# h-walk/PySlice

Hardware: AMD Instinct MI355X
Metric: slice-steps/sec (probes x frames x slices / s), potential + slice loop + exit FFT (higher is better)
Workload: dtype complex64 (f32); 1 GPU; 64-probe STEM grid, 1024x1024 grid, 200 slices, 54 MD frames per GPU (BASELINE configs[2] per-frame work), 106583 atoms, 30 mrad, 100 keV; grid=1024, slices=200, probes=64, parallelism=frames x1, world_size_checked=1, frame_slots=59, frame_batch=4

## Files before the change

### pyslice_amd/csrc/mslice.hip

```cpp
#include <hip/hip_runtime.h>

#include <algorithm>
#include <cmath>
#include <cstdarg>
#include <cstdio>
#include <cstdlib>
#include <cstring>
#include <string>
#include <type_traits>
#include <vector>

#include "../../include/mslice.h"
#include "fft_generic.h"
#include "fft_pow2.h"
#include "rowtm_pass.h"
#include "potential.h"
#include "thermal.h"
#include "phonons.h"
#include "reduce.h"
#include "stream.h"
#include "tacaw_time.h"
#include "tacaw_launch.h"
#include "tacaw_welch.h"
#include "layer_tap.h"
// ... 36 lines not shown
    }
    int reserve(msl_handle* h, size_t count) { return count <= n ? MSL_OK : alloc(h, count); }
};

struct FftPlan {
    int M = 0;
    DevBuf<float2> chirp, bfilt;
    int N = 0;
    int n_stages = 0;
    int radix[MSL_MAX_STAGES] = {0};
    DevBuf<float2> tw;
    bool ok = false;
};

enum LaunchKind { K_ROW = 0, K_COL = 1, K_OTHER = 2, K_NKINDS = 3 };

enum AxisKind { AX_NONE, AX_FOURSTEP, AX_TWO, AX_WAVE2K, AX_MIXED, AX_CONV, AX_CONV2K, AX_CONV4K, AX_GENERIC };

enum PotIfft { PI_LINES, PI_TWO, PI_CHIRPZ, PI_WAVE2K };

struct CzTables { int R = 0; DevBuf<float2> tw, tw2, bf, bw; };

struct EventSet {
    std::vector<hipEvent_t> ev;
    std::vector<int> kind;
    int used = 0;
    bool pending = false;
};

}

struct msl_handle {
    msl_config cfg{};
    hipStream_t stream = nullptr;
    std::string err;
    FftPlan plan_x, plan_y, plan_t;
    int Rx = 0, Ry = 0;
    DevBuf<float2> tw4_x, tw4_y;
    int n_cus = 256;
    int wx = 0, wy = 0, wx0 = 0, wy0 = 0;
    size_t wpix = 0;
    size_t wpitch = 0;
    size_t intensity_ld = 0;
    int bx = 1, by = 1;
    DevBuf<float2> bin_stage;
    DevBuf<float2> st_acc, st_tw; DevBuf<double2> st_s1; DevBuf<double> st_s2; DevBuf<int> st_bins;
    DevBuf<float2> st_ref; bool st_have_ref = false;
    int st_T = 0, st_F = 0; bool st_open = false;
    int64_t intensity_F = 0;
    DevBuf<char> scratch;
    bool onepass = false;
    bool scheme_b = false;
    PotIfft pot_ifft = PI_LINES;
    struct OpDir { AxisKind kind = AX_NONE, base = AX_NONE; int n = 0; int R = 0; DevBuf<float2> mtw, tw, tw2, qf, bw, ptab;
                   CzTables cz; } opx, opy;
    CzTables opt;
    int opt_T = 0;
    DevBuf<float2> tsplit_tw;
    int tsplit_T = 0;
    DevBuf<float> welch_g;
    std::vector<float> welch_g_host;
    DevBuf<float2> psiT, psi0T;
    bool need_psi0T = false;
    int keys_cap = 0;
    struct HostStage { char* buf = nullptr; size_t bytes = 0; hipEvent_t ev = nullptr; bool used = false; } stage[2];
    unsigned stage_pos = 0;
    DevBuf<float2> transT;
    int pitchT = 0;
    int debug_flags_mask = -1;
    int row_pchunk = 0;
    int pitch = 0;
    int FB = 1, cur_batch = 0;
    DevBuf<float2> psi0, psi, trans;
    DevBuf<float> V;
    DevBuf<float> intensity;
    DevBuf<float2> pxt, pyt;
    std::vector<int> layer_block;
    std::vector<int> layer_slices;
    DevBuf<float2> layers;
    float2* wf = nullptr;
    DevBuf<float2> tap, tap_cx, tap_cy;
    bool lr_on = false;
    unsigned lr_what = 0;
    int lr_bx = 1, lr_by = 1, lr_slot = 0, lr_count = 0;
    LrLayout lr_lay;
    DevBuf<float2> lr_block;
    DevBuf<double> lr_stage;
    DevBuf<uint16_t> det_mask;
    DevBuf<float> det_kx, det_ky;
    int det_n = 0, det_wy = 0;
    size_t det_K = 0;
    uint32_t det_amp = 0, det_cx = 0, det_cy = 0;
    DevBuf<uint32_t> pol_order;
    DevBuf<long long> pol_seg;
    int pol_bins = 0;
    size_t pol_K = 0;
    DevBuf<double> diff_out;
    DevBuf<double2> coh_acc;
    int64_t coh_B = 0, coh_K = 0;
    DevBuf<double> img_acc;
    int64_t img_n = 0;
    std::vector<int32_t> sm_h;
    DevBuf<int2> sm_beams;
    DevBuf<float2> sm_S, sm_c;
    int sm_fx = 0, sm_fy = 0, sm_Bm = 0;
    bool sm_open = false, sm_built = false;
// ... 806 lines not shown
            j.in = h->psiT; j.out = h->psi;
            j.trans = h->transT + toff + (size_t)k * npix; j.pl = h->pxt;
            j.in_image_stride = isB; j.out_image_stride = isA; j.in_pitch = h->pitchT; j.out_pitch = h->pitch; j.n_lines = c.ny;
            rc = launch_rowT_dir(h, h->opx, j, K_COL);
        }
        if (rc) return rc;
        if (k < nz - 1) {
            int rp = 0;
            const int order = tap_order((k & 1) ? h->opx : h->opy, j.flags, j.perm_shift, &rp);
            if ((rc = tap_step(h, k, fused_slot, groups, (k & 1) ? h->psi : h->psiT, !(k & 1), order, rp, (k & 1) ? 1 : 0))) return rc;
        }
    }
    if (nz & 1) {
        dim3 grid((c.nx + 31) / 32, (c.ny + 31) / 32, P);
        hipLaunchKernelGGL(transpose_kernel, grid, dim3(256), 0, h->stream, h->psiT, h->psi, c.ny, c.nx, h->pitchT, h->pitch, isB, isA);
        HIPCHK(h, hipGetLastError());
        if ((rc = mark_launch(h, K_OTHER))) return rc;
    }
    if (fused) {
        if (h->Ry) {
            RowJob r = row_job(h, h->psi, P, h->pitch);
            r.do_fft = true;
            if ((rc = launch_row_fast(h, r, K_OTHER))) return rc;
        } else {
            LineArgs r = row_args(h, h->psi, h->psi, P, h->pitch);
            r.fft1 = +1;
            if ((rc = launch_lines(h, h->plan_y, r, K_OTHER))) return rc;
        }
        if ((rc = epilogue_x_pass(h, fused_slot, groups))) return rc;
    }
    count_slice_loop(h, P, groups, fused, 16);
    return MSL_OK;
}

template <int R>
int launch_row2_r(msl_handle* h, Row2Job job, int kind) {
    constexpr int N = R * R, G = 256 / R;
    const size_t lds = (size_t)N * 16 + (size_t)G * R * (R + 1) * 4;
    const int per_cu = std::max(1, std::min(2, (int)((size_t)h->lds_limit / lds)));
    const int grid = chunked_grid(h, job, job.nx / G, (long long)h->n_cus * per_cu);
    hipLaunchKernelGGL(row_pass2_kernel<R>, dim3(grid), dim3(256), lds, h->stream, job);
    HIPCHK(h, hipGetLastError());
    return mark_launch(h, kind);
}

int slice_loop_onepass(msl_handle* h, int fused_slot, int groups, int first_group) {
    if (h->scheme_b) return slice_loop_onepass_b(h, fused_slot, groups, first_group);
    const msl_config& c = h->cfg;
    const int P = c.n_probes * groups, nz = c.nz;
    const size_t toff = (size_t)first_group * c.nz * c.nx * c.ny;
    const size_t npix = (size_t)c.nx * c.ny;
    const long long isA = (long long)c.nx * h->pitch, isB = (long long)c.ny * h->pitchT;
    const bool fused = fused_slot >= 0;
    int rc;
    if (nz == 1)
        HIPCHK(h, hipMemcpyAsync(h->psi, h->psi0, (size_t)P * isA * sizeof(float2), hipMemcpyDeviceToDevice, h->stream));
    if ((rc = begin_timed(h, nz + 2 + (fused ? tap_launches(h) : 0)))) return rc;
    for (int k = 0; k < nz; ++k) {
        const bool last = (k == nz - 1);
        int flags = (k > 0 ? P2_PRE_A : 0) | (!last ? P2_POST_A : 0) | ((last && fused) ? P2_POST_F : 0);
        if (h->debug_flags_mask >= 0) flags &= h->debug_flags_mask;
        if (last) {
            Row2Job j{};
            j.psi = h->psi; j.trans = h->trans + toff + (size_t)k * npix; j.py = h->pyt; j.tw = h->tw4_y;
            j.image_stride = isA; j.pitch = h->pitch; j.nx = c.nx; j.n_images = P; j.flags = flags;
            set_frame_groups(h, j, groups);
            rc = h->Ry == 32 ? launch_row2_r<32>(h, j, K_ROW) : launch_row2_r<16>(h, j, K_ROW);
            if (rc) return rc;
            break;
        }
        const bool along_y = !slice_is_transposed(h, k);
        RowTJob j{};
        if (!dbg_env("MSL_NO_INTERLEAVE") && h->debug_flags_mask < 0) flags |= (k > 0 ? P2_IN_PAIRED : 0) | (k < nz - 2 ? P2_OUT_PAIRED : 0);
        j.flags = flags; j.n_images = P;
        j.perm_shift = ((along_y ? h->Rx : h->Ry) == 32) ? 2 : 1;
        set_frame_groups(h, j, groups);
        if (along_y) {
            j.in = (k == 0) ? h->psi0 : h->psi; j.out = h->psiT;
            j.trans = h->trans + toff + (size_t)k * npix; j.pl = h->pyt; j.tw = h->tw4_y;
            j.in_image_stride = isA; j.out_image_stride = isB; j.in_pitch = h->pitch; j.out_pitch = h->pitchT; j.n_lines = c.nx;
            rc = h->Ry == 32 ? launch_rowT_r<32>(h, j, K_ROW) : launch_rowT_r<16>(h, j, K_ROW);
        } else {
            j.in = (k == 0) ? h->psi0T : h->psiT; j.out = h->psi;
            j.trans = h->transT + toff + (size_t)k * npix; j.pl = h->pxt; j.tw = h->tw4_x;
            j.in_image_stride = isB; j.out_image_stride = isA; j.in_pitch = h->pitchT; j.out_pitch = h->pitch; j.n_lines = c.ny;
            rc = h->Rx == 32 ? launch_rowT_r<32>(h, j, K_COL) : launch_rowT_r<16>(h, j, K_COL);
        }
        if (rc) return rc;
        const int order = (j.flags & P2_OUT_PAIRED) ? TAP_INTERLEAVED : TAP_NATURAL;
        if ((rc = tap_step(h, k, fused_slot, groups, along_y ? h->psiT : h->psi, along_y, order, 8 << j.perm_shift, along_y ? 0 : 1))) return rc;
    }
    if (fused && (rc = epilogue_x_pass(h, fused_slot, groups))) return rc;
    count_slice_loop(h, P, groups, fused, 16);
    return MSL_OK;
}

int ensure_atoms(msl_handle* h, size_t n, size_t rows) {
    if (rows <= h->atom_cap) return MSL_OK;
    (void)n;
    size_t cap = std::max<size_t>(rows, h->atom_cap * 3 / 2 + 1024);
    int rc;
    if ((rc = h->d_pos.alloc(h, cap * 3)) || (rc = h->d_Z.alloc(h, cap)) || (rc = h->d_key.alloc(h, cap)) || (rc = h->d_order.alloc(h, cap)) ||
        (rc = h->d_u1.alloc(h, cap)) || (rc = h->d_u2.alloc(h, cap))) return rc;
    if ((rc = h->d_ex.alloc(h, cap * (size_t)(h->cfg.nx / 2 + 1))) || (rc = h->d_ey.alloc(h, cap * (size_t)(h->cfg.ny / 2 + 1)))) return rc;
    h->atom_cap = cap;
    return MSL_OK;
}

int slice_loop(msl_handle* h, int fused_slot, int groups, int first_group) {
    if (h->onepass) return slice_loop_onepass(h, fused_slot, groups, first_group);
    const msl_config& c = h->cfg;
    const int P = c.n_probes * groups, nz = c.nz;
    const size_t npix = (size_t)c.nx * c.ny;
    const size_t toff = (size_t)first_group * c.nz * npix;
    HIPCHK(h, hipMemcpyAsync(h->psi, h->psi0, (size_t)P * c.nx * h->pitch * sizeof(float2), hipMemcpyDeviceToDevice, h->stream));
    const bool fused = fused_slot >= 0;
    int rc = begin_timed(h, 2 * nz + 2 + (fused ? tap_launches(h) : 0));
    if (rc) return rc;
    for (int z = 0; z < nz; ++z) {
        const bool last = (z == nz - 1);
        if (h->Ry) {
            RowJob r = row_job(h, h->psi, P, h->pitch);
            r.do_ifft = z > 0; r.trans = h->trans + toff + (size_t)z * npix;
            r.do_fft = (!last || fused); r.py = last ? nullptr : h->pyt;
            set_frame_groups(h, r, groups);
            if ((rc = launch_row_fast(h, r, K_ROW))) return rc;
        } else {
            LineArgs r = row_args(h, h->psi, h->psi, P, h->pitch);
            r.fft1 = (z > 0) ? -1 : 0;
            r.m1_kind = MUL_ARRAY; r.m1 = h->trans + toff + (size_t)z * npix; r.m1_ls = c.ny;
            if (groups > 1) { r.group = c.n_probes; r.m_gs = (long long)c.nz * npix; r.out_gs = (long long)c.n_probes * r.out_is; }
            if (!last) { r.fft2 = +1; r.m2_kind = MUL_VEC; r.m2 = h->pyt; }
            else if (fused) { r.fft2 = +1; }
            if ((rc = launch_lines(h, h->plan_y, r, K_ROW))) return rc;
        }
        if (!last && (rc = tap_step(h, z, fused_slot, groups, h->psi, false, TAP_NATURAL, 8, 2))) return rc;
        if (!last) {
            if (h->Rx) {
                ColJob k = col_job(h, h->psi, h->psi, P, h->pitch, h->pitch);
                k.px = h->pxt; k.flags = COL_FWD | COL_MULPX | COL_INV;
                if ((rc = launch_col_fast(h, k, K_COL))) return rc;
            } else {
                LineArgs k = col_args(h, h->psi, h->psi, P, h->pitch, h->pitch);
                k.fft1 = +1; k.m1_kind = MUL_VEC; k.m1 = h->pxt; k.fft2 = -1;
                if ((rc = launch_lines(h, h->plan_x, k, K_COL))) return rc;
// ... 135 lines not shown
                if (mG == 64) T[n + (n1 % mA) * 2 * mB + 2 * k2 + n1 / mA] = w;
                else T[n + n1 * mB + k2] = w;
            }
        if (mG == 64)
            for (int m = 0; m < mA; ++m) {
                const double a = -2.0 * M_PI * (double)m / (double)(2 * mA);
                T[2 * n + m] = make_float2(1.f, 0.f);
                T[2 * n + mA + m] = make_float2((float)cos(a), (float)sin(a));
            }
        if ((rc = upload(h, o.mtw, T))) return rc;
    }
    switch (o.base) {
    case AX_TWO: {
        std::vector<float2> t(o.R * o.R);
        for (int m = 0; m < o.R * o.R; ++m) {
            const double a = -2.0 * M_PI * (double)m / (double)n;
            t[m] = make_float2((float)cos(a), (float)sin(a));
        }
        if ((rc = make_tw4(h, o.tw, o.R)) || (rc = upload(h, o.tw2, t)) || (rc = o.ptab.alloc(h, (size_t)n))) return rc;
        break;
    }
    case AX_WAVE2K:
        if ((rc = make_wave2k_tables(h, o.tw, o.tw2))) return rc;
        break;
    case AX_CONV:
    case AX_CONV2K:
        if ((rc = make_cz_tables(h, o.cz, n)) || (rc = o.qf.alloc(h, conv_filter_entries(o)))) return rc;
        break;
    case AX_CONV4K: {
        std::vector<float2> wq(2048);
        for (int i = 0; i < 2048; ++i) {
            const double a = -2.0 * M_PI * (double)i / 4096.0;
            wq[i] = make_float2((float)cos(a), (float)sin(a));
        }
        if ((rc = make_wave2k_tables(h, o.tw, o.tw2)) || (rc = upload(h, o.bw, wq)) || (rc = o.qf.alloc(h, conv_filter_entries(o)))) return rc;
        break;
    }
    default:
        break;
    }
    auto conv = [](const msl_handle::OpDir& d) { return d.base == AX_CONV || d.base == AX_CONV2K; };
    if (!conv(o) && conv(other) && n >= 33 && n <= 1024) return make_cz_tables(h, o.cz, n);
    return MSL_OK;
}

PotIfft plan_pot_ifft(const msl_handle* h) {
    if (!h->onepass || h->V) return PI_LINES;
    if (h->opx.base == AX_WAVE2K && h->opy.base == AX_WAVE2K && h->transT) return PI_WAVE2K;
    if (h->transT && h->opx.cz.R && h->opy.cz.R) return PI_CHIRPZ;
    if (h->opx.base == AX_TWO && h->opy.base == AX_TWO) return PI_TWO;
    return PI_LINES;
}

bool pot_half_rows(const msl_handle* h) { return h->pot_ifft != PI_LINES || (h->Rx && h->Ry); }

struct PotGroup {
    int z2s[104], species[104], nsp;
    int64_t n; int32_t ax1, ax2, axs;
    int keys_per_frame;
    int cx, cy; float vscale;
    bool half_rows, sf_stream;
    int g, slot, n_slices, nkeys;
    long long rows, rows_pad;
    float2* TR; float2* TRT;
};

void drop_modes(msl_handle* h) {
    h->have_modes = false;
    h->md_basis.release(); h->md_q.release(); h->md_tau.release(); h->md_W.release(); h->md_C.release();
    h->md_M = h->md_nb = 0;
}

int map_species(msl_handle* h, const int32_t* Z, int64_t n, PotGroup& m) {
    for (int i = 0; i < 104; ++i) m.z2s[i] = -1;
    for (int64_t a = 0; a < n; ++a) {
        if (Z[a] < 1 || Z[a] > 103) return fail(h, MSL_ERR_INVALID, "msl_build_potential: atomic number %d out of 1..103", Z[a]);
        m.z2s[Z[a]] = 0;
    }
    m.nsp = 0;
    for (int z = 1; z <= 103; ++z) if (m.z2s[z] == 0) { m.z2s[z] = m.nsp; m.species[m.nsp++] = z; }
    return MSL_OK;
}

int stage_atoms(msl_handle* h, const PotGroup& p, const double* pos, const int32_t* Z, bool send_maps) {
    msl_handle::HostStage& st = h->stage[h->stage_pos++ & 1];
    if (!st.ev) HIPCHK(h, hipEventCreateWithFlags(&st.ev, hipEventDisableTiming));
    if (st.used) HIPCHK(h, hipEventSynchronize(st.ev));
    const size_t z_bytes = (size_t)p.n * sizeof(int), pos_bytes = (size_t)p.rows * 3 * sizeof(double);
    const size_t off_sp = sizeof p.z2s, off_Z = (off_sp + sizeof p.species + 7) & ~(size_t)7;
    const size_t off_pos = (off_Z + z_bytes + 7) & ~(size_t)7, need = off_pos + pos_bytes;
    if (need > st.bytes) {
        if (st.buf) (void)hipHostFree(st.buf);
        st.buf = nullptr; st.bytes = 0;
        const size_t cap = need + need / 4;
        if (hipHostMalloc((void**)&st.buf, cap, hipHostMallocDefault) != hipSuccess)
            return fail(h, MSL_ERR_NOMEM, "hipHostMalloc(%zu bytes) failed", cap);
        st.bytes = cap;
    }
    memcpy(st.buf + off_pos, pos, pos_bytes);
    if (send_maps) {
        memcpy(st.buf, p.z2s, sizeof p.z2s);
        memcpy(st.buf + off_sp, p.species, sizeof p.species);
        memcpy(st.buf + off_Z, Z, z_bytes);
        HIPCHK(h, hipMemcpyAsync(h->d_z2s, st.buf, sizeof p.z2s, hipMemcpyHostToDevice, h->stream));
        HIPCHK(h, hipMemcpyAsync(h->d_species, st.buf + off_sp, p.nsp * sizeof(int), hipMemcpyHostToDevice, h->stream));
        HIPCHK(h, hipMemcpyAsync(h->d_Z, st.buf + off_Z, z_bytes, hipMemcpyHostToDevice, h->stream));
// ... 529 lines not shown
        static int exchange_ok = -1;
        if (exchange_ok < 0) exchange_ok = rowT_selftest(h->stream);
        if (exchange_ok != 0) return bail(fail(h, MSL_ERR_HIP, "msl_create: the add-tid LDS exchange self-test failed on this device / toolchain (%d values wrong)", exchange_ok));
    }
    if ((rc = make_plan(h, h->plan_x, cfg->nx))) return bail(rc);
    if ((rc = make_plan(h, h->plan_y, cfg->ny))) return bail(rc);
    {
        hipDeviceProp_t prop;
        if (hipGetDeviceProperties(&prop, cfg->device) == hipSuccess && prop.multiProcessorCount > 0) h->n_cus = prop.multiProcessorCount;
    }
    if (cfg->fft_path == 0) {
        int ry = fast_radix(cfg->ny), rx = fast_radix(cfg->nx);
        if (ry && cfg->nx % (256 / ry) == 0) { h->Ry = ry; if ((rc = make_tw4(h, h->tw4_y, ry))) return bail(rc); }
        if (rx && cfg->ny % 16 == 0 && cfg->ny >= 32) { h->Rx = rx; if ((rc = make_tw4(h, h->tw4_x, rx))) return bail(rc); }
        { const char* e = dbg_env("MSL_ROW_PCHUNK"); if (e) h->row_pchunk = atoi(e); }
        allow_lds(h, row_pass_pf_kernel<32>);
        allow_lds(h, row_pass_pf_kernel<16>);
        allow_lds(h, col_pass_kernel<32>);
        allow_lds(h, col_pass_kernel<16>);
    }
    const size_t npix = (size_t)cfg->nx * cfg->ny;
    {
        const char* e = dbg_env("MSL_PITCH_PAD");
        int pad = e ? atoi(e) : 16;
        if (pad < 0 || (pad & 1)) pad = 16;
        h->pitch = cfg->ny + ((h->Rx || h->Ry) ? pad : 0);
    }
    {
        const char* e = dbg_env("MSL_SLICE_PATH");
        const bool want = cfg->fft_path == 0 && !(e && atoi(e) == 2);
        plan_axis_kind(h, h->opx, cfg->nx, cfg->ny, h->Rx, h->plan_x.M, want);
        plan_axis_kind(h, h->opy, cfg->ny, cfg->nx, h->Ry, h->plan_y.M, want);
        if ((rc = make_axis_tables(h, h->opx, h->opy)) || (rc = make_axis_tables(h, h->opy, h->opx))) return bail(rc);
        h->onepass = h->opx.base != AX_NONE && h->opy.base != AX_NONE;
        h->scheme_b = h->onepass && !(h->opx.kind == AX_FOURSTEP && h->opy.kind == AX_FOURSTEP);
        if (h->pitch == cfg->ny && h->onepass) h->pitch = cfg->ny + 16;
        if (h->onepass && (h->pitch & 1)) ++h->pitch;
        if (h->onepass) {
            h->pitchT = cfg->nx + 16 + (cfg->nx & 1);
            if (h->pitch - cfg->ny > 16 && !(cfg->nx & 1)) h->pitchT = cfg->nx + (h->pitch - cfg->ny);
            h->need_psi0T = !h->scheme_b && (cfg->nz % 2 == 0);
        }
        if ((rc = alloc_probe_buffers(h, cfg->n_probes))) return bail(rc);
        if (h->onepass) {
            if ((rc = h->transT.alloc(h, npix * cfg->nz * h->FB))) return bail(rc);
            { const char* ev = dbg_env("MSL_DEBUG_FLAGS_MASK"); if (ev) h->debug_flags_mask = atoi(ev); }
            allow_lds(h, row_pass2_kernel<32>);
            allow_lds(h, row_pass2_kernel<16>);
        }
    }
    if ((rc = h->trans.alloc(h, npix * cfg->nz * h->FB))) return bail(rc);
    if (cfg->keep_potential && (rc = h->V.alloc(h, npix * cfg->nz))) return bail(rc);
    h->pot_ifft = plan_pot_ifft(h);
    if (cfg->n_frames > 0) {
        if ((h->bx > 1 || h->by > 1) && (rc = h->bin_stage.alloc(h, (size_t)h->wx * h->wy * cfg->n_probes * h->FB))) return bail(rc);
        if ((rc = h->layers.alloc(h, layer_block_elems(h)))) return bail(rc);
        h->wf = h->layers;
        if (hipMemsetAsync(h->wf, 0, layer_block_elems(h) * sizeof(float2), h->stream) != hipSuccess)
            return bail(fail(h, MSL_ERR_HIP, "memset failed"));
    }
    if ((rc = h->pxt.alloc(h, (size_t)cfg->nx)) || (rc = h->pyt.alloc(h, (size_t)cfg->ny)) || (rc = h->tap_cx.alloc(h, (size_t)cfg->nx)) ||
        (rc = h->tap_cy.alloc(h, (size_t)cfg->ny)) || (rc = h->d_lo.alloc(h, (size_t)cfg->nz)) || (rc = h->d_hi.alloc(h, (size_t)cfg->nz)) ||
        (rc = h->d_abcd.alloc(h, (size_t)103 * 12)) || (rc = h->d_z2s.alloc(h, (size_t)104)) || (rc = h->d_species.alloc(h, (size_t)104)) ||
        (rc = fill_propagator(h))) return bail(rc);
    *out = h;
    return MSL_OK;
}

int msl_destroy(msl_handle* h) {
    if (!h) return MSL_OK;
    (void)hipSetDevice(h->cfg.device);
    if (h->stream) (void)hipStreamSynchronize(h->stream);
    for (auto& s : h->ring) for (auto e : s.ev) (void)hipEventDestroy(e);
    for (auto& st : h->stage) { if (st.ev) (void)hipEventDestroy(st.ev); if (st.buf) (void)hipHostFree(st.buf); }
    const hipStream_t stream = h->stream;
    delete h;
    if (stream) (void)hipStreamDestroy(stream);
    return MSL_OK;
}

int msl_set_kirkland(msl_handle* h, const double* abcd) {
    if (!h || !abcd) return fail(h, MSL_ERR_INVALID, "msl_set_kirkland: null argument");
    HIPCHK(h, hipSetDevice(h->cfg.device));
    HIPCHK(h, hipMemcpyAsync(h->d_abcd, abcd, 103 * 12 * sizeof(double), hipMemcpyHostToDevice, h->stream));
    HIPCHK(h, hipStreamSynchronize(h->stream));
    h->have_kirkland = true;
    h->n_species = 0;
    h->ff_n = 0;
    return MSL_OK;
}

int msl_set_slices(msl_handle* h, const double* lo, const double* hi) {
    if (!h || !lo || !hi) return fail(h, MSL_ERR_INVALID, "msl_set_slices: null argument");
    for (int s = 0; s < h->cfg.nz; ++s)
        if (!(hi[s] > lo[s]) || (s > 0 && lo[s] < lo[s - 1]))
            return fail(h, MSL_ERR_INVALID, "msl_set_slices: edges must be increasing with hi>lo (slice %d)", s);
    HIPCHK(h, hipSetDevice(h->cfg.device));
    HIPCHK(h, hipMemcpyAsync(h->d_lo, lo, h->cfg.nz * sizeof(double), hipMemcpyHostToDevice, h->stream));
    HIPCHK(h, hipMemcpyAsync(h->d_hi, hi, h->cfg.nz * sizeof(double), hipMemcpyHostToDevice, h->stream));
    HIPCHK(h, hipStreamSynchronize(h->stream));
    h->have_slices = true;
    return MSL_OK;
}

int msl_set_beam(msl_handle* h, double wavelength, double sigma, double dz) {
    if (!h) return fail(h, MSL_ERR_INVALID, "null handle");
// ... 1736 lines not shown
```

### pyslice_amd/csrc/rowt_pass.h

```cpp
#pragma once
#include <type_traits>
#include <utility>
#include <hip/hip_runtime.h>
#include "fft_regs.h"
#include "kernel_util.h"

#ifndef MSL_ABL2
#define MSL_ABL2 0
#endif
#ifndef MSL_TW_LDS
#define MSL_TW_LDS 0
#endif
#ifndef MSL_DIT_LCH
#define MSL_DIT_LCH 8
#endif
#ifndef MSL_DIT_FENCE
#define MSL_DIT_FENCE 0
#endif
#ifndef MSL_STAGGER
#define MSL_STAGGER 4
#endif
#define MSL_IC(x) std::integral_constant<int, (x)>{}

namespace msl {

enum { P2_PRE_A = 1, P2_POST_A = 2, P2_POST_F = 4, P2_IN_PAIRED = 8, P2_OUT_PAIRED = 16 };

struct RowTJob {
    const float2* in;
    float2* out;
    const float2* trans;
    const float2* pl;
    const float2* tw;
    const float2* tw2;
    long long in_image_stride, out_image_stride;
    int in_pitch, out_pitch, n_lines, n_images, flags, pchunk;
    int t_group;
    unsigned t_magic;
    long long t_stride;
    const float2* bf;
    const float2* bw;
    int n_line;
    int perm_shift;
#ifdef MSL_CLOCK
    unsigned long long* clk;
#endif
};

template <typename Job>
__device__ __forceinline__ long long frame_off(const Job& job, int p) {
    if (job.t_group <= 0) return 0;
    const unsigned up = (unsigned)__builtin_amdgcn_readfirstlane(p);
    const unsigned f = job.t_group == 1 ? up : __umulhi(up, job.t_magic);
    return (long long)f * job.t_stride;
}


template <int R>
__device__ __forceinline__ void exchange_addtid(float2 (&v)[R], const float* scratch_base, unsigned wave_scratch, int ln, int lane64) {
    static_assert(64 % R == 0 && R % 4 == 0, "R-lane groups inside one wave; rows are read four floats at a time");
    constexpr int PW = 68;
    if constexpr (MSL_ABL2 & 4) return;
    const float* rd = scratch_base + ln * PW + (lane64 / R) * R;
    asm volatile("s_mov_b32 m0, %0\n\ts_nop 1" :: "s"(wave_scratch) : "memory");
#pragma unroll
    for (int k1 = 0; k1 < R; ++k1) asm volatile("ds_write_addtid_b32 %0 offset:%1" :: "v"(v[k1].x), "n"(k1 * PW * 4) : "memory");
    wave_lds_fence();
#pragma unroll
    for (int g = 0; g < R / 4; ++g) {
        const float4 q = *reinterpret_cast<const float4*>(rd + 4 * g);
        v[4 * g].x = q.x; v[4 * g + 1].x = q.y; v[4 * g + 2].x = q.z; v[4 * g + 3].x = q.w;
    }
    wave_lds_fence();
    asm volatile("s_mov_b32 m0, %0\n\ts_nop 1" :: "s"(wave_scratch) : "memory");
#pragma unroll
    for (int k1 = 0; k1 < R; ++k1) asm volatile("ds_write_addtid_b32 %0 offset:%1" :: "v"(v[k1].y), "n"(k1 * PW * 4) : "memory");
    wave_lds_fence();
#pragma unroll
    for (int g = 0; g < R / 4; ++g) {
        const float4 q = *reinterpret_cast<const float4*>(rd + 4 * g);
        v[4 * g].y = q.x; v[4 * g + 1].y = q.y; v[4 * g + 2].y = q.z; v[4 * g + 3].y = q.w;
    }
    wave_lds_fence();
}

template <int R, bool INV, int WMODE, int STRIDE, int C0, typename TabPtr, int... J>
__device__ __forceinline__ void dit_leaf_chunk(const float2* in, float2* v, TabPtr tab, int ln, std::integer_sequence<int, J...>) {
    constexpr int LR = dit_leaf_radix(R), C = R / LR;
    float2 w[sizeof...(J)][4];
    if constexpr (MSL_ABL2 & 16) {
        ((w[J][0] = tab[ln], w[J][1] = tab[ln], w[J][2] = tab[ln], w[J][3] = tab[ln]), ...);
    } else {
        ((w[J][0] = tab[(C0 + J) * STRIDE + ln], w[J][1] = tab[(C0 + J + C) * STRIDE + ln]), ...);
        if constexpr (LR == 4) ((w[J][2] = tab[(C0 + J + 2 * C) * STRIDE + ln], w[J][3] = tab[(C0 + J + 3 * C) * STRIDE + ln]), ...);
    }
    (dit_leaf<R, INV, WMODE, C0 + J>(in, v, w[J]), ...);
    (pin(v[C0 + J]), ...); (pin(v[C0 + J + C]), ...);
    if constexpr (LR == 4) { (pin(v[C0 + J + 2 * C]), ...); (pin(v[C0 + J + 3 * C]), ...); }
    __builtin_amdgcn_sched_barrier(0);
}
template <int R, bool INV, int WMODE, int STRIDE, int CH, int C0, typename TabPtr>
__device__ __forceinline__ void dit_leaf_chunks(const float2* in, float2* v, TabPtr tab, int ln) {
    if constexpr (C0 < dit_leaf_count(R)) {
        dit_leaf_chunk<R, INV, WMODE, STRIDE, C0>(in, v, tab, ln, std::make_integer_sequence<int, CH>{});
        dit_leaf_chunks<R, INV, WMODE, STRIDE, CH, C0 + CH>(in, v, tab, ln);
    }
}

template <int R, bool INV, int WMODE, int K, int I>
__device__ __forceinline__ void dit_leaves_regs_part(const float2* in, float2* v, const float2* w) {
    if constexpr (I < K) {
        constexpr int LR = dit_leaf_radix(R);
        float2 ww[4];
        ww[0] = w[I]; ww[1] = w[I + K];
        if constexpr (LR == 4) { ww[2] = w[I + 2 * K]; ww[3] = w[I + 3 * K]; }
        dit_leaf<R, INV, WMODE, I>(in, v, ww);
        dit_leaves_regs_part<R, INV, WMODE, K, I + 1>(in, v, w);
    }
}
constexpr int rowT_tw_reg_leaves(int R, int FL) { return (!MSL_TW_LDS && R == 32 && FL >= 0) ? 8 : 0; }
constexpr int ROWT_TW_REG_LCH = 4;

template <int R, int LINES, bool IN_P, bool OUT_P, int FL>
__global__ void __launch_bounds__(LINES * R, (R == 16) ? 3 : 2) rowT_pass_kernel(RowTJob job) {
    constexpr int N = R * R;
    constexpr int NT = LINES * R;
    constexpr int CS = (R * R + 33) / 32 * 32 + 2;
    constexpr int TPS = LINES / 2;
    constexpr int POS_PER_IT = NT / TPS;
    constexpr int NIT = N / POS_PER_IT;
    constexpr int TWK = rowT_tw_reg_leaves(R, FL), LRW = dit_leaf_radix(R);
    constexpr bool TWR = TWK > 0;
    constexpr int LCH0 = TWR ? ROWT_TW_REG_LCH : MSL_DIT_LCH;
    constexpr int LCHL = LCH0 < dit_leaf_count(R) ? LCH0 : dit_leaf_count(R);
    constexpr int FN = MSL_DIT_FENCE;
    static_assert(LINES == 16, "16 lines = 128-byte transposed segments (8 lines / 64 bytes measured 1.6x slower)");
    static_assert(dit_leaf_count(R) % LCHL == 0 && TWK % LCHL == 0 && TWK < dit_leaf_count(R), "whole chunks");
    extern __shared__ __attribute__((aligned(16))) char smem_raw[];
    float2* tw = reinterpret_cast<float2*>(smem_raw);
    float2* pl = tw + N;
    float2* tile = pl + N;
    const int tid = threadIdx.x;
    for (int i = tid; i < N; i += NT) { tw[i] = job.tw[i]; pl[i] = job.pl[i]; }
    __syncthreads();
    const int grp = tid / R, ln = tid % R;
    float2 twr[TWR ? LRW * TWK : 1];
    if constexpr (TWR) {
#pragma unroll
        for (int i = 0; i < LRW * TWK; ++i) twr[i] = tw[((i % TWK) + (i / TWK) * dit_leaf_count(R)) * R + ln];
        pin_all(twr);
    }
    const int q = tid % TPS, r0 = tid / TPS;
    const int l64 = tid & 63;
    float2* myrow = tile + grp * CS;
    const float* wscr = reinterpret_cast<const float*>(tile + (grp - grp % (64 / R)) * CS);
    const unsigned wscr_lds = __builtin_amdgcn_readfirstlane((unsigned)(size_t)(tile + (grp - grp % (64 / R)) * CS));
    const int lblocks = job.n_lines / LINES;
    const int PC = job.pchunk;
    const int pchunks = (job.n_images + PC - 1) / PC;
    const int n_items = lblocks * pchunks;
    const bool pre_a = (MSL_ABL2 & 8) ? false : FL >= 0 ? (FL & P2_PRE_A) != 0 : (job.flags & P2_PRE_A) != 0;
    const bool post_a = (MSL_ABL2 & 8) ? false : FL >= 0 ? (FL & P2_POST_A) != 0 : (job.flags & P2_POST_A) != 0;
    const int step_lb = (int)gridDim.x / pchunks, step_pc = (int)gridDim.x % pchunks;
    auto line_of = [&](int lbb) {
        if constexpr (OUT_P) {
            const int sh = job.perm_shift;
            return (((lbb >> sh) * 2 + (grp & 1)) << (sh + 3)) + 8 * (lbb & ((1 << sh) - 1)) + (grp >> 1);
        } else {
            return lbb * LINES + grp;
        }
    };
    auto line_ptr = [&](int lbb, int pcc, int kk) {
        return job.in + (long long)(pcc * PC + kk) * job.in_image_stride + (long long)line_of(lbb) * job.in_pitch;
    };
    auto load_regs = [&](float2 (&dst)[R], const float2* r, auto lo_c, auto hi_c) {
        constexpr int LO = decltype(lo_c)::value, HI = decltype(hi_c)::value;
        if constexpr (IN_P) {
            static_assert(LO % 2 == 0 && HI % 2 == 0, "register pairs");
#pragma unroll
            for (int jp = LO / 2; jp < HI / 2; ++jp) {
                const msl_f4v t = __builtin_nontemporal_load(reinterpret_cast<const msl_f4v*>(r + (2 * R * jp + 2 * ln)));
                dst[2 * jp] = make_float2(t.x, t.y); dst[2 * jp + 1] = make_float2(t.z, t.w);
            }
        } else {
#pragma unroll
            for (int j = LO; j < HI; ++j) dst[j] = ld_stream(r + (j * R + ln));
        }
    };
    int item = blockIdx.x;
    int lb = item / pchunks, pc = item - lb * pchunks, k = 0;
    float2 vn[R];
    if (item < n_items) load_regs(vn, line_ptr(lb, pc, 0), MSL_IC(0), MSL_IC(R));
    __builtin_amdgcn_s_waitcnt(0x0F70);
    float2 tv[R];
#ifdef MSL_CLOCK
    const unsigned long long clk0 = __builtin_amdgcn_s_memtime(), rt0 = __builtin_amdgcn_s_memrealtime();
#endif
    while (item < n_items) {
        if constexpr (MSL_STAGGER > 0)
            for (int i = __builtin_amdgcn_readfirstlane(tid >> 6) & 3; i > 0; --i) __builtin_amdgcn_s_sleep(MSL_STAGGER);
        float2 v[R];
        const int p = pc * PC + k;
        const int cur_lb = lb;
        if (k == 0) {
            const float2* trow = job.trans + frame_off(job, pc * PC) + (long long)line_of(lb) * N;
#pragma unroll
            for (int j = 0; j < R; ++j) tv[j] = ld_stream(trow + j * R + ln);
        }
        int nitem = item, nlb = lb, npc = pc, nk = k + 1;
        if (nk >= min(PC, job.n_images - pc * PC)) {
            nk = 0; nitem = item + (int)gridDim.x; nlb = lb + step_lb; npc = pc + step_pc;
            if (npc >= pchunks) { npc -= pchunks; ++nlb; }
        }
        const bool more = nitem < n_items;
        const float2* nptr = line_ptr(more ? nlb : lb, more ? npc : pc, more ? nk : k);
        auto pfx = [&](auto i_c) {
            constexpr int I = decltype(i_c)::value;
            constexpr int LO = (R * I / 16) & ~1, HI = (R * (I + 1) / 16) & ~1;
            if constexpr (HI > LO && !(MSL_ABL2 & 1)) {
                __builtin_amdgcn_sched_barrier(0);
                load_regs(vn, nptr, MSL_IC(LO), MSL_IC(HI));
                __builtin_amdgcn_sched_barrier(0);
            }
        };
#define MSL_HALF_TAB(INV, WM, TAB, I0) do { dit_leaf_chunks<R, INV, WM, R, LCHL, 0>(v, v, TAB, ln); pfx(MSL_IC(I0)); \
                                            dit_upper<R, INV, FN>(v); pin_all(v); pfx(MSL_IC((I0) + 1)); } while (0)
#define MSL_HALF_TW(INV, WM, I0) do { \
            if constexpr (TWR) { dit_leaves_regs_part<R, INV, WM, TWK, 0>(v, v, twr); \
                                 dit_leaf_chunks<R, INV, WM, R, LCHL, TWK>(v, v, tw, ln); pin_all(v); pfx(MSL_IC(I0)); \
                                 dit_upper<R, INV, FN>(v); pin_all(v); pfx(MSL_IC((I0) + 1)); } \
            else MSL_HALF_TAB(INV, WM, tw, I0); } while (0)
        if (pre_a) {
            dit_leaves_plain<R, false, 0>(vn, v); pin_all(v);
            pfx(MSL_IC(0));
            dit_upper<R, false, FN>(v); pin_all(v);
            pfx(MSL_IC(1));
            exchange_addtid<R>(v, wscr, wscr_lds, ln, l64);
            MSL_HALF_TW(false, 1, 2);
            MSL_HALF_TAB(true, 1, pl, 4);
            exchange_addtid<R>(v, wscr, wscr_lds, ln, l64);
            MSL_HALF_TW(true, 2, 6);
        } else {
#pragma unroll
            for (int j = 0; j < R; ++j) v[j] = vn[j];
            pin_all(v);
            pfx(MSL_IC(0)); pfx(MSL_IC(1)); pfx(MSL_IC(2)); pfx(MSL_IC(3)); pfx(MSL_IC(4)); pfx(MSL_IC(5)); pfx(MSL_IC(6)); pfx(MSL_IC(7));
        }
        if (post_a) {
            dit_leaves_regs<R, false, 1, 0>(v, v, tv); pin_all(v);
            pfx(MSL_IC(8));
            dit_upper<R, false, FN>(v); pin_all(v);
            pfx(MSL_IC(9));
            exchange_addtid<R>(v, wscr, wscr_lds, ln, l64);
            MSL_HALF_TW(false, 1, 10);
            MSL_HALF_TAB(true, 1, pl, 12);
            exchange_addtid<R>(v, wscr, wscr_lds, ln, l64);
            MSL_HALF_TW(true, 2, 14);
        } else {
#pragma unroll
            for (int j = 0; j < R; ++j) v[j] = cmulf(v[j], tv[j]);
            pfx(MSL_IC(8)); pfx(MSL_IC(9)); pfx(MSL_IC(10)); pfx(MSL_IC(11)); pfx(MSL_IC(12)); pfx(MSL_IC(13)); pfx(MSL_IC(14)); pfx(MSL_IC(15));
        }
#undef MSL_HALF_TW
#undef MSL_HALF_TAB
        if constexpr (MSL_ABL2 & 32) {
            float acc = 0.f;
#pragma unroll
            for (int j = 0; j < R; ++j) acc += v[j].x + v[j].y;
            if (acc == 1.2345e-30f) job.out[tid] = make_float2(acc, acc);
            item = nitem; lb = nlb; pc = npc; k = nk;
            continue;
        }
        wave_lds_fence();
#pragma unroll
        for (int j = 0; j < R; ++j) myrow[j * R + ln] = v[j];
        lds_barrier();
        float2* dst = job.out + (long long)p * job.out_image_stride + cur_lb * LINES;
        int off0 = 2 * q + r0 * job.out_pitch;
        asm volatile("" : "+v"(off0));
        const int ostep = POS_PER_IT * job.out_pitch;
#pragma unroll
        for (int i = 0; i < NIT; ++i) {
            const int pos = r0 + POS_PER_IT * i;
            const float2 a = tile[(2 * q) * CS + pos], b = tile[(2 * q + 1) * CS + pos];
#if MSL_ABL2 & 2
            if (a.x == 1.2345e-30f)
#endif
            st_stream(dst + (off0 + i * ostep), a.x, a.y, b.x, b.y);
        }
        lds_barrier();
        item = nitem; lb = nlb; pc = npc; k = nk;
    }
#ifdef MSL_CLOCK
    if (tid == 0 && job.clk) {
        job.clk[2 * blockIdx.x] = __builtin_amdgcn_s_memtime() - clk0;
        job.clk[2 * blockIdx.x + 1] = __builtin_amdgcn_s_memrealtime() - rt0;
    }
#endif
}

constexpr size_t rowT_lds_bytes(int R) { return ((size_t)2 * R * R + (size_t)16 * ((R * R + 33) / 32 * 32 + 2)) * 8; }

bool rowT_launch(int R, const RowTJob& job, int grid, size_t lds_limit, hipStream_t stream);
int rowT_selftest(hipStream_t stream);

}
```

### pyslice_amd/csrc/slice_pass.hip

```cpp
#include "rowt_pass.h"

namespace msl {

template <int R, bool IN_P, bool OUT_P, int FL>
static bool launch_one(const RowTJob& job, int grid, size_t lds_limit, hipStream_t stream) {
    (void)hipFuncSetAttribute((const void*)rowT_pass_kernel<R, 16, IN_P, OUT_P, FL>, hipFuncAttributeMaxDynamicSharedMemorySize, (int)lds_limit);
    hipLaunchKernelGGL((rowT_pass_kernel<R, 16, IN_P, OUT_P, FL>), dim3(grid), dim3(16 * R), rowT_lds_bytes(R), stream, job);
    return true;
}

template <int R>
static bool launch_r(const RowTJob& job, int grid, size_t lds_limit, hipStream_t stream) {
    const bool in_p = job.flags & P2_IN_PAIRED, out_p = job.flags & P2_OUT_PAIRED;
    const int fl = job.flags & (P2_PRE_A | P2_POST_A);
    if (in_p && out_p && fl == 3) return launch_one<R, true, true, 3>(job, grid, lds_limit, stream);
    if (!in_p && out_p && fl == 2) return launch_one<R, false, true, 2>(job, grid, lds_limit, stream);
    if (in_p && !out_p && fl == 1) return launch_one<R, true, false, 1>(job, grid, lds_limit, stream);
    if (in_p && !out_p && fl == 3) return launch_one<R, true, false, 3>(job, grid, lds_limit, stream);
    if (!in_p && !out_p && fl == 3) return launch_one<R, false, false, 3>(job, grid, lds_limit, stream);
    if (!in_p && !out_p) return launch_one<R, false, false, -1>(job, grid, lds_limit, stream);
    return false;
}

bool rowT_launch(int R, const RowTJob& job, int grid, size_t lds_limit, hipStream_t stream) {
    if (R == 32) return launch_r<32>(job, grid, lds_limit, stream);
    if (R == 16) return launch_r<16>(job, grid, lds_limit, stream);
    return false;
}

template <int R>
__global__ void __launch_bounds__(64) exchange_selftest_kernel(int* bad) {
    __shared__ __attribute__((aligned(16))) float scr[R * 68];
    const int lane = threadIdx.x, g = lane / R, l = lane % R;
    float2 v[R];
#pragma unroll
    for (int j = 0; j < R; ++j) v[j] = make_float2((float)(1000 * g + 32 * j + l), -(float)(1000 * g + 32 * j + l));
    const unsigned base = __builtin_amdgcn_readfirstlane((unsigned)(size_t)scr);
    exchange_addtid<R>(v, scr, base, l, lane);
    int wrong = 0;
#pragma unroll
    for (int j = 0; j < R; ++j) {
        const float want = (float)(1000 * g + 32 * l + j);
        wrong += (v[j].x != want) + (v[j].y != -want);
    }
    if (wrong) atomicAdd(bad, wrong);
}

int rowT_selftest(hipStream_t stream) {
    int* bad = nullptr;
    if (hipMalloc(&bad, sizeof(int)) != hipSuccess) return -1;
    int host = -1;
    bool ok = hipMemsetAsync(bad, 0, sizeof(int), stream) == hipSuccess;
    if (ok) {
        hipLaunchKernelGGL(exchange_selftest_kernel<32>, dim3(1), dim3(64), 0, stream, bad);
        hipLaunchKernelGGL(exchange_selftest_kernel<16>, dim3(1), dim3(64), 0, stream, bad);
        ok = hipGetLastError() == hipSuccess && hipMemcpyAsync(&host, bad, sizeof(int), hipMemcpyDeviceToHost, stream) == hipSuccess &&
             hipStreamSynchronize(stream) == hipSuccess;
    }
    (void)hipFree(bad);
    return ok ? host : -1;
}

}
```

Baseline: 248,000 slice-steps/s.

## Run the exit FFT as transposed row passes writing shifted frames directly

When the layout allows it, the last slice now runs through the transposed row-pass kernel in a forward-only mode (A-finish then forward FFT). A new exit-only row pass then performs the final x-axis FFT and writes each probe into its frame slot with an fftshift folded into the store addressing. This replaces the old row_pass2 last slice followed by a separate epilogue x pass, aiming to save memory traffic and a non-transposed pass over the grid. It adds new template instantiations and index logic for frame groups and the shift, and it is gated off under debug or binning configurations.

```diff
diff --git a/pyslice_amd/csrc/mslice.hip b/pyslice_amd/csrc/mslice.hip
--- a/pyslice_amd/csrc/mslice.hip
+++ b/pyslice_amd/csrc/mslice.hip
@@ -112,6 +112,7 @@
     bool onepass = false;
     bool scheme_b = false;
     PotIfft pot_ifft = PI_LINES;
+    bool exit_passes = false;
     struct OpDir { AxisKind kind = AX_NONE, base = AX_NONE; int n = 0; int R = 0; DevBuf<float2> mtw, tw, tw2, qf, bw, ptab;
                    CzTables cz; } opx, opy;
     CzTables opt;
@@ -1024,6 +1025,7 @@
     const size_t npix = (size_t)c.nx * c.ny;
     const long long isA = (long long)c.nx * h->pitch, isB = (long long)c.ny * h->pitchT;
     const bool fused = fused_slot >= 0;
+    const bool tail = fused && h->exit_passes;
     int rc;
     if (nz == 1)
         HIPCHK(h, hipMemcpyAsync(h->psi, h->psi0, (size_t)P * isA * sizeof(float2), hipMemcpyDeviceToDevice, h->stream));
@@ -1032,7 +1034,7 @@
         const bool last = (k == nz - 1);
         int flags = (k > 0 ? P2_PRE_A : 0) | (!last ? P2_POST_A : 0) | ((last && fused) ? P2_POST_F : 0);
         if (h->debug_flags_mask >= 0) flags &= h->debug_flags_mask;
-        if (last) {
+        if (last && !tail) {
             Row2Job j{};
             j.psi = h->psi; j.trans = h->trans + toff + (size_t)k * npix; j.py = h->pyt; j.tw = h->tw4_y;
             j.image_stride = isA; j.pitch = h->pitch; j.nx = c.nx; j.n_images = P; j.flags = flags;
@@ -1043,7 +1045,7 @@
         }
         const bool along_y = !slice_is_transposed(h, k);
         RowTJob j{};
-        if (!dbg_env("MSL_NO_INTERLEAVE") && h->debug_flags_mask < 0) flags |= (k > 0 ? P2_IN_PAIRED : 0) | (k < nz - 2 ? P2_OUT_PAIRED : 0);
+        if (!dbg_env("MSL_NO_INTERLEAVE") && h->debug_flags_mask < 0) flags |= (k > 0 ? P2_IN_PAIRED : 0) | ((tail || k < nz - 2) ? P2_OUT_PAIRED : 0);
         j.flags = flags; j.n_images = P;
         j.perm_shift = ((along_y ? h->Rx : h->Ry) == 32) ? 2 : 1;
         set_frame_groups(h, j, groups);
@@ -1059,10 +1061,20 @@
             rc = h->Rx == 32 ? launch_rowT_r<32>(h, j, K_COL) : launch_rowT_r<16>(h, j, K_COL);
         }
         if (rc) return rc;
+        if (last) break;
         const int order = (j.flags & P2_OUT_PAIRED) ? TAP_INTERLEAVED : TAP_NATURAL;
         if ((rc = tap_step(h, k, fused_slot, groups, along_y ? h->psiT : h->psi, along_y, order, 8 << j.perm_shift, along_y ? 0 : 1))) return rc;
     }
-    if (fused && (rc = epilogue_x_pass(h, fused_slot, groups))) return rc;
+    if (tail) {
+        RowTJob j{};
+        j.flags = P2_EXIT | P2_IN_PAIRED; j.n_images = P;
+        set_frame_groups(h, j, groups);
+        j.in = h->psiT; j.out = h->wf + (size_t)fused_slot * h->wpitch; j.tw = h->tw4_x;
+        j.pl = h->pxt;
+        j.in_image_stride = isB; j.in_pitch = h->pitchT; j.n_lines = c.ny;
+        j.out_image_stride = (long long)c.n_frames * h->wpitch; j.out_group_stride = (long long)h->wpitch; j.out_pitch = h->wy;
+        if ((rc = h->Rx == 32 ? launch_rowT_r<32>(h, j, K_COL) : launch_rowT_r<16>(h, j, K_COL))) return rc;
+    } else if (fused && (rc = epilogue_x_pass(h, fused_slot, groups))) return rc;
     count_slice_loop(h, P, groups, fused, 16);
     return MSL_OK;
 }
@@ -1304,6 +1316,15 @@
     return PI_LINES;
 }
 
+bool plan_exit_passes(const msl_handle* h) {
+    const msl_config& c = h->cfg;
+    if (!h->onepass || h->scheme_b || !h->Rx || !h->Ry || c.nz < 2 || c.n_frames <= 0) return false;
+    if (h->wx != c.nx || h->wy != c.ny || h->bx > 1 || h->by > 1) return false;
+    if (c.nx % 32 || c.ny % 32) return false;
+    if (h->debug_flags_mask >= 0 || dbg_env("MSL_NO_INTERLEAVE")) return false;
+    return !dbg_env("MSL_OLD_TAIL");
+}
+
 bool pot_half_rows(const msl_handle* h) { return h->pot_ifft != PI_LINES || (h->Rx && h->Ry); }
 
 struct PotGroup {
@@ -1939,6 +1960,7 @@
     if ((rc = h->trans.alloc(h, npix * cfg->nz * h->FB))) return bail(rc);
     if (cfg->keep_potential && (rc = h->V.alloc(h, npix * cfg->nz))) return bail(rc);
     h->pot_ifft = plan_pot_ifft(h);
+    h->exit_passes = plan_exit_passes(h);
     if (cfg->n_frames > 0) {
         if ((h->bx > 1 || h->by > 1) && (rc = h->bin_stage.alloc(h, (size_t)h->wx * h->wy * cfg->n_probes * h->FB))) return bail(rc);
         if ((rc = h->layers.alloc(h, layer_block_elems(h)))) return bail(rc);
diff --git a/pyslice_amd/csrc/rowt_pass.h b/pyslice_amd/csrc/rowt_pass.h
--- a/pyslice_amd/csrc/rowt_pass.h
+++ b/pyslice_amd/csrc/rowt_pass.h
@@ -24,7 +24,7 @@
 
 namespace msl {
 
-enum { P2_PRE_A = 1, P2_POST_A = 2, P2_POST_F = 4, P2_IN_PAIRED = 8, P2_OUT_PAIRED = 16 };
+enum { P2_PRE_A = 1, P2_POST_A = 2, P2_POST_F = 4, P2_IN_PAIRED = 8, P2_OUT_PAIRED = 16, P2_EXIT = 32 };
 
 struct RowTJob {
     const float2* in;
@@ -42,6 +42,7 @@
     const float2* bw;
     int n_line;
     int perm_shift;
+    long long out_group_stride;
 #ifdef MSL_CLOCK
     unsigned long long* clk;
 #endif
@@ -122,7 +123,7 @@
 constexpr int ROWT_TW_REG_LCH = 4;
 
 template <int R, int LINES, bool IN_P, bool OUT_P, int FL>
-__global__ void __launch_bounds__(LINES * R, (R == 16) ? 3 : 2) rowT_pass_kernel(RowTJob job) {
+__device__ __forceinline__ void rowT_pass_body(const RowTJob& job) {
     constexpr int N = R * R;
     constexpr int NT = LINES * R;
     constexpr int CS = (R * R + 33) / 32 * 32 + 2;
@@ -131,6 +132,10 @@
     constexpr int NIT = N / POS_PER_IT;
     constexpr int TWK = rowT_tw_reg_leaves(R, FL), LRW = dit_leaf_radix(R);
     constexpr bool TWR = TWK > 0;
+    constexpr bool EXIT = FL >= 0 && (FL & P2_EXIT) != 0, POST_F = FL >= 0 && (FL & P2_POST_F) != 0;
+    static_assert(!EXIT || FL == P2_EXIT, "the exit pass is the forward transform alone");
+    static_assert(!POST_F || FL == (P2_PRE_A | P2_POST_F), "the forward-only second half follows an A-finish");
+    static_assert(!EXIT || !OUT_P, "the frame slots are in natural order");
     constexpr int LCH0 = TWR ? ROWT_TW_REG_LCH : MSL_DIT_LCH;
     constexpr int LCHL = LCH0 < dit_leaf_count(R) ? LCH0 : dit_leaf_count(R);
     constexpr int FN = MSL_DIT_FENCE;
@@ -202,7 +207,7 @@
         float2 v[R];
         const int p = pc * PC + k;
         const int cur_lb = lb;
-        if (k == 0) {
+        if (!EXIT && k == 0) {
             const float2* trow = job.trans + frame_off(job, pc * PC) + (long long)line_of(lb) * N;
 #pragma unroll
             for (int j = 0; j < R; ++j) tv[j] = ld_stream(trow + j * R + ln);
@@ -230,13 +235,21 @@
                                  dit_leaf_chunks<R, INV, WM, R, LCHL, TWK>(v, v, tw, ln); pin_all(v); pfx(MSL_IC(I0)); \
                                  dit_upper<R, INV, FN>(v); pin_all(v); pfx(MSL_IC((I0) + 1)); } \
             else MSL_HALF_TAB(INV, WM, tw, I0); } while (0)
-        if (pre_a) {
+        if constexpr (EXIT) {
             dit_leaves_plain<R, false, 0>(vn, v); pin_all(v);
             pfx(MSL_IC(0));
             dit_upper<R, false, FN>(v); pin_all(v);
             pfx(MSL_IC(1));
             exchange_addtid<R>(v, wscr, wscr_lds, ln, l64);
             MSL_HALF_TW(false, 1, 2);
+            pfx(MSL_IC(4)); pfx(MSL_IC(5)); pfx(MSL_IC(6)); pfx(MSL_IC(7));
+        } else if (pre_a) {
+            dit_leaves_plain<R, false, 0>(vn, v); pin_all(v);
+            pfx(MSL_IC(0));
+            dit_upper<R, false, FN>(v); pin_all(v);
+            pfx(MSL_IC(1));
+            exchange_addtid<R>(v, wscr, wscr_lds, ln, l64);
+            MSL_HALF_TW(false, 1, 2);
             MSL_HALF_TAB(true, 1, pl, 4);
             exchange_addtid<R>(v, wscr, wscr_lds, ln, l64);
             MSL_HALF_TW(true, 2, 6);
@@ -246,13 +259,23 @@
             pin_all(v);
             pfx(MSL_IC(0)); pfx(MSL_IC(1)); pfx(MSL_IC(2)); pfx(MSL_IC(3)); pfx(MSL_IC(4)); pfx(MSL_IC(5)); pfx(MSL_IC(6)); pfx(MSL_IC(7));
         }
-        if (post_a) {
+        if constexpr (EXIT) {
+            pfx(MSL_IC(8)); pfx(MSL_IC(9)); pfx(MSL_IC(10)); pfx(MSL_IC(11)); pfx(MSL_IC(12)); pfx(MSL_IC(13)); pfx(MSL_IC(14)); pfx(MSL_IC(15));
+        } else if constexpr (POST_F) {
             dit_leaves_regs<R, false, 1, 0>(v, v, tv); pin_all(v);
             pfx(MSL_IC(8));
             dit_upper<R, false, FN>(v); pin_all(v);
             pfx(MSL_IC(9));
             exchange_addtid<R>(v, wscr, wscr_lds, ln, l64);
             MSL_HALF_TW(false, 1, 10);
+            pfx(MSL_IC(12)); pfx(MSL_IC(13)); pfx(MSL_IC(14)); pfx(MSL_IC(15));
+        } else if (post_a) {
+            dit_leaves_regs<R, false, 1, 0>(v, v, tv); pin_all(v);
+            pfx(MSL_IC(8));
+            dit_upper<R, false, FN>(v); pin_all(v);
+            pfx(MSL_IC(9));
+            exchange_addtid<R>(v, wscr, wscr_lds, ln, l64);
+            MSL_HALF_TW(false, 1, 10);
             MSL_HALF_TAB(true, 1, pl, 12);
             exchange_addtid<R>(v, wscr, wscr_lds, ln, l64);
             MSL_HALF_TW(true, 2, 14);
@@ -275,7 +298,20 @@
 #pragma unroll
         for (int j = 0; j < R; ++j) myrow[j * R + ln] = v[j];
         lds_barrier();
-        float2* dst = job.out + (long long)p * job.out_image_stride + cur_lb * LINES;
+        float2* dst;
+        if constexpr (EXIT) {
+            long long obase = (long long)p * job.out_image_stride;
+            if (job.t_group > 0) {
+                const unsigned up = (unsigned)__builtin_amdgcn_readfirstlane(p);
+                const unsigned f = job.t_group == 1 ? up : __umulhi(up, job.t_magic);
+                obase = (long long)(up - f * (unsigned)job.t_group) * job.out_image_stride + (long long)f * job.out_group_stride;
+            }
+            int col = cur_lb * LINES + job.n_lines / 2;
+            if (col >= job.n_lines) col -= job.n_lines;
+            dst = job.out + obase + col;
+        } else {
+            dst = job.out + (long long)p * job.out_image_stride + cur_lb * LINES;
+        }
         int off0 = 2 * q + r0 * job.out_pitch;
         asm volatile("" : "+v"(off0));
         const int ostep = POS_PER_IT * job.out_pitch;
@@ -286,7 +322,7 @@
 #if MSL_ABL2 & 2
             if (a.x == 1.2345e-30f)
 #endif
-            st_stream(dst + (off0 + i * ostep), a.x, a.y, b.x, b.y);
+            st_stream(dst + (off0 + (EXIT ? i ^ (NIT / 2) : i) * ostep), a.x, a.y, b.x, b.y);
         }
         lds_barrier();
         item = nitem; lb = nlb; pc = npc; k = nk;
@@ -299,6 +335,17 @@
 #endif
 }
 
+template <int R, int LINES, bool IN_P, bool OUT_P, int FL>
+__global__ void __launch_bounds__(LINES * R, (R == 16) ? 3 : 2) rowT_pass_kernel(RowTJob job) {
+    rowT_pass_body<R, LINES, IN_P, OUT_P, FL>(job);
+}
+
+template <int R, int LINES, bool IN_P, bool OUT_P, int FL>
+__global__ void __launch_bounds__(LINES * R, (R == 16) ? 3 : 2) rowT_tail_kernel(RowTJob job) {
+    static_assert(FL == P2_EXIT || FL == (P2_PRE_A | P2_POST_F), "tail forms only");
+    rowT_pass_body<R, LINES, IN_P, OUT_P, FL>(job);
+}
+
 constexpr size_t rowT_lds_bytes(int R) { return ((size_t)2 * R * R + (size_t)16 * ((R * R + 33) / 32 * 32 + 2)) * 8; }
 
 bool rowT_launch(int R, const RowTJob& job, int grid, size_t lds_limit, hipStream_t stream);
diff --git a/pyslice_amd/csrc/slice_pass.hip b/pyslice_amd/csrc/slice_pass.hip
--- a/pyslice_amd/csrc/slice_pass.hip
+++ b/pyslice_amd/csrc/slice_pass.hip
@@ -9,10 +9,19 @@
     return true;
 }
 
+template <int R, bool IN_P, bool OUT_P, int FL>
+static bool launch_tail(const RowTJob& job, int grid, size_t lds_limit, hipStream_t stream) {
+    (void)hipFuncSetAttribute((const void*)rowT_tail_kernel<R, 16, IN_P, OUT_P, FL>, hipFuncAttributeMaxDynamicSharedMemorySize, (int)lds_limit);
+    hipLaunchKernelGGL((rowT_tail_kernel<R, 16, IN_P, OUT_P, FL>), dim3(grid), dim3(16 * R), rowT_lds_bytes(R), stream, job);
+    return true;
+}
+
 template <int R>
 static bool launch_r(const RowTJob& job, int grid, size_t lds_limit, hipStream_t stream) {
     const bool in_p = job.flags & P2_IN_PAIRED, out_p = job.flags & P2_OUT_PAIRED;
     const int fl = job.flags & (P2_PRE_A | P2_POST_A);
+    if (job.flags & P2_EXIT) return in_p && !out_p ? launch_tail<R, true, false, P2_EXIT>(job, grid, lds_limit, stream) : false;
+    if (job.flags & P2_POST_F) return in_p && out_p && fl == P2_PRE_A ? launch_tail<R, true, true, P2_PRE_A | P2_POST_F>(job, grid, lds_limit, stream) : false;
     if (in_p && out_p && fl == 3) return launch_one<R, true, true, 3>(job, grid, lds_limit, stream);
     if (!in_p && out_p && fl == 2) return launch_one<R, false, true, 2>(job, grid, lds_limit, stream);
     if (in_p && !out_p && fl == 1) return launch_one<R, true, false, 1>(job, grid, lds_limit, stream);
```

Result: no change. 248,400 slice-steps/s (median of 6 runs) (+0.2%).
